# ZHENGXi-git/TC-VIML

Hardware: NVIDIA B200
Metric: linearized_factors_per_s (higher is better)
Workload: dtype f64

## Files before the change

tc-viml_b200/csrc/assemble2.cuh:

```cuda
#pragma once

namespace stream {

constexpr int PMAX = 12;
constexpr int FMAXP = 4096;
constexpr int PT = 64;
constexpr int PT_MAX = 512;
constexpr int TASK_T = 180;
constexpr int TASK_F = 24;
constexpr int LTASK = 32;
constexpr int AW = 4;
constexpr int LACC_W = 14;
constexpr int STAGE_D = 1024;
constexpr int LACC_D = TASK_F * LACC_W;
constexpr int WORK_D = STAGE_D + LACC_D + 192;

struct PlanPtrs {
  int4* hdr;
  int4* tasks;
  uint32_t* slots;
  uint32_t* finfo;
  uint32_t* lslots;
  int* any_irregular;
};

__host__ __device__ inline int task_base(int a0_rel, int w, int F) { return a0_rel / 64 + w * (F / TASK_F + PMAX + 4); }

__device__ __forceinline__ int warp_incl_scan(int v, int lane) {
#pragma unroll
  for (int d = 1; d < 32; d <<= 1) {
    const int t = __shfl_up_sync(0xffffffffu, v, d);
    if (lane >= d) v += t;
  }
  return v;
}

__global__ void __launch_bounds__(PT_MAX) plan_kernel(LinearizeArgs A, PlanPtrs PL) {
  extern __shared__ __align__(16) unsigned char plan_raw[];
  __shared__ int gcount[PMAX + 2], grun[PMAX + 2], lcount[PMAX + 1], lrun[PMAX + 1];
  __shared__ int s_bad, s_big, s_ntasks, s_nlslots;
  const int tid = threadIdx.x, lane = tid & 31, warp = tid >> 5, w = blockIdx.x;
  const int P = A.P, F = A.F, NTH = (int)blockDim.x;
  uint32_t* fmask = reinterpret_cast<uint32_t*>(plan_raw);
  uint32_t* fanchor = fmask + F;
  uint32_t* cexcl = fanchor + F;
  uint16_t* ford = reinterpret_cast<uint16_t*>(cexcl + F + 1);
  uint16_t* fid = ford + ((F + 1) & ~1);
  const int a0 = A.pf_window_offset[w], nf = A.pf_window_offset[w + 1] - a0;
  const int b0 = A.NL > 0 ? A.lf_window_offset[w] : 0, nl = A.NL > 0 ? A.lf_window_offset[w + 1] - b0 : 0;
  const int a0r = a0 - (int)A.pf_begin, b0r = b0 - (int)A.lf_begin;
  for (int f = tid; f < F; f += NTH) fmask[f] = 0u, fanchor[f] = 0xffu;
  for (int e = tid; e < F * P; e += NTH) fid[e] = 0xffff;
  if (tid < PMAX + 2) gcount[tid] = 0;
  if (tid < PMAX + 1) lcount[tid] = 0;
  if (tid == 0) s_bad = s_big = (nf > 65534 || nl > 65534 || nf < 0 || nl < 0) ? 1 : 0, s_ntasks = 0, s_nlslots = 0;
  __syncthreads();
  const int nfs = s_big ? 0 : nf;
  for (int k = tid; k < nfs; k += NTH) {
    const uint32_t ix = A.pf_idx[a0 + k];
    const int i = ix & 0xff, j = (ix >> 8) & 0xff, l = ix >> 16;
    if (i >= P || j >= P || l >= F || i == j) {
      s_bad = 1;
      continue;
    }
    const uint32_t old = atomicOr(&fmask[l], 1u << j);
    const uint32_t an = atomicCAS(&fanchor[l], 0xffu, (uint32_t)i);
    if (((old >> j) & 1u) || (an != 0xffu && an != (uint32_t)i)) s_bad = 1;
    fid[l * P + j] = (uint16_t)k;
  }
  __syncthreads();
  if (s_bad) {
    if (tid == 0) {
      PL.hdr[w] = make_int4(0, 0, 1, 0);
      atomicOr(PL.any_irregular, 1);
    }
    return;
  }
  uint32_t* lsl = PL.lslots + 2 * (size_t)b0r;
  if (warp == 0) {
    for (int f0 = 0; f0 < F; f0 += 32) {
      const int f = f0 + lane;
      const int key = f < F ? (fanchor[f] == 0xffu ? P : (int)fanchor[f]) : 64 + lane;
      const unsigned m = __match_any_sync(0xffffffffu, key);
      if (f < F && (m & ((1u << lane) - 1u)) == 0u) gcount[key] += __popc(m);
      __syncwarp();
    }
    {
      const int c = lane <= P ? gcount[lane] : 0;
      const int inc = warp_incl_scan(c, lane);
      if (lane <= P) grun[lane] = inc - c;
    }
    __syncwarp();
    for (int f0 = 0; f0 < F; f0 += 32) {
      const int f = f0 + lane;
      const int key = f < F ? (fanchor[f] == 0xffu ? P : (int)fanchor[f]) : 64 + lane;
      const unsigned m = __match_any_sync(0xffffffffu, key);
      const int rank = __popc(m & ((1u << lane) - 1u));
      if (f < F) ford[grun[key] + rank] = (uint16_t)f;
      __syncwarp();
      if (f < F && rank == 0) grun[key] += __popc(m);
      __syncwarp();
    }
    int carry = 0;
    for (int p0 = 0; p0 < F; p0 += 32) {
      const int p = p0 + lane;
      const int c = p < F ? __popc(fmask[ford[p]]) : 0;
      const int inc = warp_incl_scan(c, lane);
      if (p < F) cexcl[p] = (uint32_t)(carry + inc - c);
      carry += __shfl_sync(0xffffffffu, inc, 31);
    }
    if (lane == 0) cexcl[F] = (uint32_t)carry;
    __syncwarp();
    const int tb = task_base(a0r, w, F);
    int pos = 0, t = 0;
    bool at_group_start = true;
    while (pos < F) {
      const int p = pos + lane;
      const int c = p < F ? (int)(cexcl[p + 1] - cexcl[p]) : 0x10000;
      const int inc = warp_incl_scan(c, lane);
      const unsigned okm = __ballot_sync(0xffffffffu, inc <= TASK_T && p < F && lane < TASK_F);
      int n = okm == 0xffffffffu ? 32 : __ffs(~okm) - 1;
      n = max(n, 1);
      n = min(n, F - pos);
      const int an = p < F ? (fanchor[ford[p]] == 0xffu ? P : (int)fanchor[ford[p]]) : -1;
      const unsigned same = __ballot_sync(0xffffffffu, an == __shfl_sync(0xffffffffu, an, 0));
      const int na = same == 0xffffffffu ? 33 : __ffs(~same) - 1;
      int excl = 0;
      if (na <= n) {
        n = na;
        excl = at_group_start ? 1 : 0;
        at_group_start = true;
      } else {
        at_group_start = false;
      }
      if (lane == 0) PL.tasks[tb + t] = make_int4(2 * (int)cexcl[pos], 0, pos, n | (excl << 16));
      pos += n, ++t;
    }
    if (lane == 0) s_ntasks = t;
  } else if (warp == 1 && nl > 0) {
    bool bad = false;
    for (int k0 = 0; k0 < nl; k0 += 32) {
      const int k = k0 + lane;
      int key = k < nl ? A.lf_frame[b0 + k] : 64 + lane;
      if (k < nl && (key < 0 || key >= P)) bad = true, key = 96 + lane;
      const unsigned m = __match_any_sync(0xffffffffu, key);
      if (k < nl && key < P && (m & ((1u << lane) - 1u)) == 0u) lcount[key] += __popc(m);
      __syncwarp();
    }
    if (__any_sync(0xffffffffu, bad)) {
      if (lane == 0) s_bad = 1;
    } else {
      const int c = lane < P ? ((lcount[lane] + 1) & ~1) : 0;
      const int inc = warp_incl_scan(c, lane);
      if (lane < P) {
        lrun[lane] = inc - c;
        if (lcount[lane] & 1) lsl[inc - 1] = 0xffffu | ((uint32_t)lane << 16);
      }
      if (lane == 31) s_nlslots = inc;
      __syncwarp();
      for (int k0 = 0; k0 < nl; k0 += 32) {
        const int k = k0 + lane;
        const int key = k < nl ? A.lf_frame[b0 + k] : 64 + lane;
        const unsigned m = __match_any_sync(0xffffffffu, key);
        const int rank = __popc(m & ((1u << lane) - 1u));
        if (k < nl) lsl[lrun[key] + rank] = (uint32_t)k | ((uint32_t)key << 16);
        __syncwarp();
        if (k < nl && rank == 0) lrun[key] += __popc(m);
        __syncwarp();
      }
    }
  }
  __syncthreads();
  if (s_bad) {
    if (tid == 0) {
      PL.hdr[w] = make_int4(0, 0, 1, 0);
      atomicOr(PL.any_irregular, 1);
    }
    return;
  }
  const int tb = task_base(a0r, w, F), nt = s_ntasks;
  uint32_t* sl_w = PL.slots + 2 * (size_t)a0r;
  for (int t = warp; t < nt; t += NTH / 32) {
    int4 tk = PL.tasks[tb + t];
    const int p = tk.z + lane;
    const bool on = lane < (tk.w & 0xffff);
    const int l = on ? ford[p] : 0;
    const uint32_t m = on ? fmask[l] : 0u;
    const int an = (on && m) ? (int)fanchor[l] : 0xff;
    if (on) PL.finfo[(size_t)w * F + p] = (uint32_t)l | (m << 16) | ((uint32_t)(an & 15) << 28);
    uint32_t* sl = sl_w + tk.x;
    int off = 0;
    const unsigned lt = (1u << lane) - 1u;
    unsigned im = __reduce_or_sync(0xffffffffu, an < P ? 1u << an : 0u);
    while (im) {
      const int i = __ffs(im) - 1;
      im &= im - 1;
      unsigned jm = __reduce_or_sync(0xffffffffu, an == i ? m : 0u);
      while (jm) {
        const int j = __ffs(jm) - 1;
        jm &= jm - 1;
        const bool mine = an == i && ((m >> j) & 1u);
        const unsigned b = __ballot_sync(0xffffffffu, mine);
        const int n = __popc(b);
        const uint32_t key = ((uint32_t)i << 21) | ((uint32_t)j << 25);
        if (mine) sl[off + __popc(b & lt)] = (uint32_t)fid[l * P + j] | ((uint32_t)lane << 16) | key;
        if ((n & 1) && lane == 0) sl[off + n] = 0xffffu | key;
        off += (n + 1) & ~1;
      }
    }
    if (lane == 0) PL.tasks[tb + t].y = off;
  }
  if (tid == 0) PL.hdr[w] = make_int4(nt, s_nlslots, 0, 0);
}

enum Kind { K_LL = 0, K_HH, K_LH, K_LE, K_HE, K_EE, K_BL, K_BH, K_BE, K_NKIND };

struct Tables {
  uint32_t seg[128];
  uint32_t lo[64];
  uint32_t ee[32];
  uint32_t line[32];
};

constexpr uint32_t tab_entry(int R, int C, int kind, int off, bool neg) {
  const int tile = (R < 8 && C < 8) ? 0 : (R < 8 ? 1 : 2);
  return 0x80000000u | (uint32_t)(tile * 64 + (R & 7) * 8 + (C & 7)) | ((uint32_t)kind << 8) | ((uint32_t)off << 12) |
         (neg ? (1u << 18) : 0u);
}

constexpr int col_type(int c) { return c < 3 ? 0 : (c < 6 ? 1 : (c < 9 ? 2 : (c < 15 ? 3 : 4))); }
constexpr int col_sub(int c) { return c < 3 ? c : (c < 6 ? c - 3 : (c < 9 ? c - 6 : (c < 15 ? c - 9 : 0))); }

constexpr Tables make_tables() {
  Tables T{};
  int ns = 0, nlo = 0, nli = 0, nee = 0;
  constexpr int kind_order[K_NKIND] = {K_LL, K_LE, K_BL, K_EE, K_BE, K_HH, K_HE, K_BH, K_LH};
  for (int ko = 0; ko < K_NKIND; ++ko)
    for (int off = 0; off < 36; ++off) {
      const int kind = kind_order[ko];
      const bool vec = kind >= K_BL;
      if (vec && off >= 6) continue;
      const int dr = vec ? off : off / 6, dc = vec ? 0 : off % 6;
      for (int R = 0; R < 16; ++R)
        for (int C = R; C < 16; ++C) {
          const int tr = col_type(R), tc = col_type(C), r = col_sub(R), c = col_sub(C);
          bool hit = false, neg = false;
          if (tr == 0 && tc == 0) {
            if (kind == K_LL || kind == K_HH) hit = dr == r && dc == c;
            if (kind == K_LH) hit = dr == r && dc == c, neg = true;
          } else if (tr == 0 && tc == 1) {
            if (kind == K_LL) hit = dr == r && dc == 3 + c;
            if (kind == K_LH) hit = dr == 3 + c && dc == r, neg = true;
          } else if (tr == 0 && tc == 2) {
            if (kind == K_LH) hit = dr == r && dc == 3 + c;
            if (kind == K_HH) hit = dr == r && dc == 3 + c, neg = true;
          } else if (tr == 0 && tc == 3) {
            if (kind == K_LE) hit = dr == r && dc == c;
            if (kind == K_HE) hit = dr == r && dc == c, neg = true;
          } else if (tr == 0 && tc == 4) {
            if (kind == K_BL) hit = dr == r;
            if (kind == K_BH) hit = dr == r, neg = true;
          } else if (tr == 1 && tc == 1) {
            if (kind == K_LL) hit = dr == 3 + r && dc == 3 + c;
          } else if (tr == 1 && tc == 2) {
            if (kind == K_LH) hit = dr == 3 + r && dc == 3 + c;
          } else if (tr == 1 && tc == 3) {
            if (kind == K_LE) hit = dr == 3 + r && dc == c;
          } else if (tr == 1 && tc == 4) {
            if (kind == K_BL) hit = dr == 3 + r;
          } else if (tr == 2 && tc == 2) {
            if (kind == K_HH) hit = dr == 3 + r && dc == 3 + c;
          } else if (tr == 2 && tc == 3) {
            if (kind == K_HE) hit = dr == 3 + r && dc == c;
          } else if (tr == 2 && tc == 4) {
            if (kind == K_BH) hit = dr == 3 + r;
          } else if (tr == 3 && tc == 3) {
            if (kind == K_EE) hit = dr == r && dc == c;
          } else if (tr == 3 && tc == 4) {
            if (kind == K_BE) hit = dr == r;
          }
          if (!hit) continue;
          const bool per_segment = kind == K_HH || kind == K_LH || kind == K_HE || kind == K_BH;
          if (per_segment) {
            T.seg[ns++] = tab_entry(R, C, kind, off, neg);
          } else if (kind == K_EE || kind == K_BE) {
            T.ee[nee++] = tab_entry(R, C, kind, off, neg);
          } else {
            T.lo[nlo++] = tab_entry(R, C, kind, off, neg);
          }
        }
    }
  for (int r = 0; r < 6; ++r)
    for (int c = r; c < 6; ++c) T.line[nli++] = tab_entry(r, c, K_LL, r * 6 + c, false);
  for (int r = 0; r < 6; ++r) T.line[nli++] = tab_entry(r, 6, K_BL, r, false);
  return T;
}
__device__ const Tables g_tables = make_tables();
static_assert(make_tables().seg[95] != 0u && make_tables().seg[96] == 0u, "63 hi-role + 33 (lo, hi) per-segment destinations = three full rounds");
static_assert(make_tables().lo[62] != 0u && make_tables().lo[63] == 0u, "63 per-anchor destinations");
static_assert(make_tables().ee[26] != 0u && make_tables().ee[27] == 0u, "27 extrinsic destinations");
static_assert(make_tables().line[26] != 0u && make_tables().line[27] == 0u, "27 line destinations");


__device__ __forceinline__ void dmma(double& d0, double& d1, double a, double b) {
  asm volatile("mma.sync.aligned.m8n8k4.row.col.f64.f64.f64.f64 {%0,%1}, {%2}, {%3}, {%0,%1};"
               : "+d"(d0), "+d"(d1)
               : "d"(a), "d"(b));
}

__device__ __forceinline__ int blk(int br, int bc, int NB) { return br * NB - (br * (br - 1)) / 2 + (bc - br); }

__device__ __forceinline__ int swz(int f) { return ((f & 1) << 2) ^ ((f >> 1) & 3); }

struct Dest {
  int src;
  int off;
  int kind;
  unsigned sign;
};
__device__ __forceinline__ Dest decode(uint32_t e) {
  Dest d;
  d.src = (e >> 31) ? (int)(e & 0xff) : -1;
  d.off = (e >> 12) & 63;
  d.kind = (e >> 8) & 15;
  d.sign = ((e >> 18) & 1u) << 31;
  return d;
}
template <int ROUNDS>
__device__ __forceinline__ void scatter(const double* __restrict__ patch, const Dest* tab, double* __restrict__ Hc,
                                        int mybase, bool store_lh = false) {
  double v[ROUNDS];
  double* dst[ROUNDS];
#pragma unroll
  for (int r = 0; r < ROUNDS; ++r) {
    const int base = __shfl_sync(0xffffffffu, mybase, tab[r].kind);
    dst[r] = Hc + base + tab[r].off;
    const double x = patch[tab[r].src >= 0 ? tab[r].src : 0];
    v[r] = __hiloint2double(__double2hiint(x) ^ (int)tab[r].sign, __double2loint(x));
  }
#pragma unroll
  for (int r = 0; r < ROUNDS; ++r) {
    if (tab[r].src >= 0) {
      if (store_lh && tab[r].kind == K_LH) *dst[r] = v[r];
      else atomicAdd(dst[r], v[r]);
    }
  }
}

__device__ __forceinline__ int kind_base(int rs, int cs, bool isb, int lo, int hi, int NB, int boff) {
  const int e = NB - 1;
  const int x = rs == 0 ? lo : (rs == 1 ? hi : e), y = cs == 0 ? lo : (cs == 1 ? hi : e);
  return isb ? boff + 6 * x : blk(x, y, NB) * 36;
}

__device__ __forceinline__ void put_patch(double* __restrict__ patch, int lane, const double (&G)[6]) {
  double2* p2 = reinterpret_cast<double2*>(patch);
  const int o = (lane >> 2) * 4 + (lane & 3);
  p2[o] = make_double2(G[0], G[1]);
  p2[32 + o] = make_double2(G[2], G[3]);
  p2[64 + o] = make_double2(G[4], G[5]);
}

template <bool MODE_A>
__global__ void __maxnreg__(168) assemble_kernel(LinearizeArgs A, PlanPtrs PL, int use_tma) {
  extern __shared__ __align__(16) unsigned char asm_raw[];
  __shared__ int s_next;
  constexpr int NT = AW * 32;
  const int tid = threadIdx.x, lane = tid & 31, warp = tid >> 5, w = blockIdx.x;
  const int P = A.P, F = A.F, D = A.D, NB = P + 1;
  const int nblk = NB * (NB + 1) / 2, boff = nblk * 36;
  const int hc_n = (boff + D + 1) & ~1;
  const int cstride = P * kPoseCache + kExCache;
  double* __restrict__ Hc = reinterpret_cast<double*>(asm_raw);
  double* __restrict__ cache = Hc + hc_n;
  double* __restrict__ work0 = cache + cstride;
  double* __restrict__ stage = work0 + warp * WORK_D;
  double* __restrict__ lacc = stage + STAGE_D;
  double* __restrict__ patch = lacc + LACC_D;

  const int4 hdr = PL.hdr[w];
  const int a0 = A.pf_window_offset[w];
  const int b0 = A.NL > 0 ? A.lf_window_offset[w] : 0;
  double* __restrict__ Hpp = A.out.H_pp + (size_t)w * D * D;
  double* __restrict__ Hlp = A.out.H_lp + (size_t)w * F * D;
  double* __restrict__ Hll = A.out.H_ll + (size_t)w * F;
  double* __restrict__ bp = A.out.b_p + (size_t)w * D;
  double* __restrict__ bl = A.out.b_l + (size_t)w * F;
  const double2* __restrict__ gc = reinterpret_cast<const double2*>(A.cache + (size_t)w * cstride);
  double2 cpre[3];
#pragma unroll
  for (int q = 0; q < 3; ++q) cpre[q] = tid + q * NT < cstride / 2 ? gc[tid + q * NT] : make_double2(0.0, 0.0);
  uint32_t traw[7];
#pragma unroll
  for (int r = 0; r < 3; ++r) traw[r] = g_tables.seg[32 * r + lane];
#pragma unroll
  for (int r = 0; r < 2; ++r) traw[3 + r] = g_tables.lo[32 * r + lane];
  traw[5] = g_tables.ee[lane], traw[6] = g_tables.line[lane];
  if (hdr.z) {
    for (int e = tid; e < D * D; e += NT) Hpp[e] = 0.0;
    for (int e = tid; e < F * D; e += NT) Hlp[e] = 0.0;
    for (int e = tid; e < F; e += NT) Hll[e] = 0.0, bl[e] = 0.0;
    for (int e = tid; e < D; e += NT) bp[e] = 0.0;
    return;
  }
  {
    double2* z = reinterpret_cast<double2*>(Hc);
    for (int e = tid; e < hc_n / 2; e += NT) z[e] = make_double2(0.0, 0.0);
    double2* c2 = reinterpret_cast<double2*>(cache);
#pragma unroll
    for (int q = 0; q < 3; ++q)
      if (tid + q * NT < cstride / 2) c2[tid + q * NT] = cpre[q];
    for (int e = tid + 3 * NT; e < cstride / 2; e += NT) c2[e] = gc[e];
  }
  if (tid == 0) s_next = 0;
  Dest tab_seg[3], tab_lo[2], tab_ee[1], tab_line[1];
#pragma unroll
  for (int r = 0; r < 3; ++r) tab_seg[r] = decode(traw[r]);
#pragma unroll
  for (int r = 0; r < 2; ++r) tab_lo[r] = decode(traw[3 + r]);
  tab_ee[0] = decode(traw[5]);
  tab_line[0] = decode(traw[6]);
  const int kb_rs = lane < K_NKIND ? (0x24904 >> (2 * lane)) & 3 : 0, kb_cs = lane < K_NKIND ? (0xA94 >> (2 * lane)) & 3 : 0;
  const bool kb_isb = lane >= K_BL && lane < K_NKIND;
  __syncthreads();

  const int ntask = hdr.x, nlsl = hdr.y, nltask = (nlsl + LTASK - 1) / LTASK;
  const int tb = task_base(a0 - (int)A.pf_begin, w, F);
  const uint32_t* __restrict__ sl_w = PL.slots + 2 * (size_t)(a0 - (int)A.pf_begin);
  const uint32_t* __restrict__ lsl_w = PL.lslots + 2 * (size_t)(b0 - (int)A.lf_begin);
  const int g = lane >> 2, kk = lane & 3;
  const int gx = g ^ ((kk >> 1) << 2);
  const double* __restrict__ frag0 = stage + (kk >> 1) * 32 + (kk & 1);
  const unsigned full = 0xffffffffu;
  const int upr = 3 * NB;
  const int ru1 = 32 + (lane & 7), rb0 = (lane * 11) >> 5, rb1 = (ru1 * 43) >> 7;
  const int rp0 = lane - 3 * rb0, rp1 = ru1 - 3 * rb1;

  double E[2] = {0.0, 0.0};
  for (;;) {
    int t = 0;
    if (lane == 0) t = atomicAdd(&s_next, 1);
    t = __shfl_sync(full, t, 0);
    if (t >= ntask + nltask) break;
    if (t < ntask) {
      const int4 tk = PL.tasks[tb + t];
      const int n_slots = tk.y, n_feats = tk.w & 0xffff;
      const bool excl = (tk.w >> 16) != 0;
      const uint32_t fi = lane < n_feats ? PL.finfo[(size_t)w * F + tk.z + lane] : 0u;
      {
        double2* z = reinterpret_cast<double2*>(lacc);
        for (int q = lane; q < LACC_D / 2; q += 32) z[q] = make_double2(0.0, 0.0);
      }
      __syncwarp();
      const uint32_t* __restrict__ sl = sl_w + tk.x;
      double G[6] = {0, 0, 0, 0, 0, 0}, R[4] = {0, 0, 0, 0};
      uint32_t nsw = lane < n_slots ? sl[lane] : 0xffffu;
      for (int c0 = 0; c0 < n_slots; c0 += 32) {
        const uint32_t sw_ = nsw;
        nsw = c0 + 32 + lane < n_slots ? sl[c0 + 32 + lane] : 0xffffu;
        const bool valid = (sw_ & 0xffffu) != 0xffffu;
        const int lf = (sw_ >> 16) & 31;
        {
          const int i = (sw_ >> 21) & 15, j = (sw_ >> 25) & 15;
          const int l = __shfl_sync(full, fi, lf) & 0xffff;
          PointJac J;
          if (valid) {
            const int64_t k = (int64_t)a0 + (sw_ & 0xffffu);
            const double4 ob = reinterpret_cast<const double4*>(A.pf_obs)[k];
            const double piz = A.pf_pts_i_z ? A.pf_pts_i_z[k] : 1.0;
            const double lam = A.inv_depth[(size_t)w * F + l];
            eval_point(A, cache, i, j, lam, ob.x, ob.y, piz, ob.z, ob.w, J);
            if (MODE_A) {
              if (A.out.pf_residual) reinterpret_cast<double2*>(A.out.pf_residual)[k] = make_double2(J.r[0], J.r[1]);
              if (A.out.pf_jac_pose_i) store_jac7(A.out.pf_jac_pose_i + 14 * k, J.a);
              if (A.out.pf_jac_pose_j) store_jac7(A.out.pf_jac_pose_j + 14 * k, J.b);
              if (A.out.pf_jac_ex) store_jac7(A.out.pf_jac_ex + 14 * k, J.c);
              if (A.out.pf_jac_feat) reinterpret_cast<double2*>(A.out.pf_jac_feat)[k] = make_double2(J.d[0], J.d[1]);
            }
            double2* row = reinterpret_cast<double2*>(Hlp + (size_t)l * D + 6 * j);
            row[0] = make_double2(J.d[0] * J.b[0][0] + J.d[1] * J.b[1][0], J.d[0] * J.b[0][1] + J.d[1] * J.b[1][1]);
            row[1] = make_double2(J.d[0] * J.b[0][2] + J.d[1] * J.b[1][2], J.d[0] * J.b[0][3] + J.d[1] * J.b[1][3]);
            row[2] = make_double2(J.d[0] * J.b[0][4] + J.d[1] * J.b[1][4], J.d[0] * J.b[0][5] + J.d[1] * J.b[1][5]);
          } else {
#pragma unroll
            for (int c = 0; c < 6; ++c) J.a[0][c] = J.a[1][c] = J.b[0][c] = J.b[1][c] = J.c[0][c] = J.c[1][c] = 0.0;
            J.r[0] = J.r[1] = J.d[0] = J.d[1] = 0.0;
          }
          {
            const bool swp = i > j;
            const int sx = swz(lane);
            double2* rec = reinterpret_cast<double2*>(stage) + lane * 16;
#pragma unroll
            for (int c = 0; c < 6; ++c) rec[c ^ sx] = swp ? make_double2(J.b[0][c], J.b[1][c]) : make_double2(J.a[0][c], J.a[1][c]);
#pragma unroll
            for (int c = 0; c < 3; ++c)
              rec[(6 + c) ^ sx] = swp ? make_double2(J.a[0][3 + c], J.a[1][3 + c]) : make_double2(J.b[0][3 + c], J.b[1][3 + c]);
#pragma unroll
            for (int c = 0; c < 6; ++c) rec[(9 + c) ^ sx] = make_double2(J.c[0][c], J.c[1][c]);
            rec[15 ^ sx] = make_double2(J.r[0], J.r[1]);
          }
          {
            const unsigned grp = __match_any_sync(full, valid ? lf : 32 + lane);
            const int rank = __popc(grp & ((1u << lane) - 1u));
            const int rounds = __reduce_max_sync(full, valid ? __popc(grp) : 0);
            double v[LACC_W];
#pragma unroll
            for (int c = 0; c < 6; ++c) {
              v[c] = J.d[0] * J.a[0][c] + J.d[1] * J.a[1][c];
              v[6 + c] = J.d[0] * J.c[0][c] + J.d[1] * J.c[1][c];
            }
            v[12] = J.d[0] * J.d[0] + J.d[1] * J.d[1];
            v[13] = J.d[0] * J.r[0] + J.d[1] * J.r[1];
            double2* __restrict__ la = reinterpret_cast<double2*>(lacc + lf * LACC_W);
            for (int r = 0; r < rounds; ++r) {
              if (valid && rank == r) {
#pragma unroll
                for (int c = 0; c < LACC_W / 2; ++c) {
// ... 4 lines not shown
              }
              __syncwarp();
            }
          }
        }
        __syncwarp();
        const uint32_t key = sw_ >> 21;
        uint32_t nk = __shfl_down_sync(full, key, 1);
        const uint32_t nk31 = __shfl_sync(full, nsw >> 21, 0);
        if (lane == 31) nk = nk31;
        if (c0 + lane + 1 >= n_slots) nk = 0xffffffffu;
        const unsigned bnd = __ballot_sync(full, key != nk);
        const int nks = min(16, (n_slots - c0) >> 1);
        int s = 0;
        while (s < nks) {
          const unsigned rem = bnd >> (2 * s + 1);
          const int q_end = rem ? ((__ffs(rem) - 1) >> 1) : 32;
          const bool ends = s + q_end < nks;
          const int s_end = ends ? s + q_end + 1 : nks;
#pragma unroll 2
          for (; s < s_end; ++s) {
            const double* __restrict__ p = frag0 + s * 64 + 2 * (gx ^ (s & 3));
            const double u0 = p[0], u1 = p[16];
            dmma(G[0], G[1], u0, u0);
            dmma(G[2], G[3], u0, u1);
            dmma(G[4], G[5], u1, u1);
          }
          if (ends) {
            const int la_ = 2 * s - 2;
            const uint32_t kseg = __shfl_sync(full, key, la_), knext = __shfl_sync(full, nk, la_ + 1);
            const int si = kseg & 15, sj = (kseg >> 4) & 15;
            const int lo = min(si, sj), hi = max(si, sj);
            const int mybase = kind_base(kb_rs, kb_cs, kb_isb, lo, hi, NB, boff);
            put_patch(patch, lane, G);
            __syncwarp();
            scatter<3>(patch, tab_seg, Hc, mybase, excl);
#pragma unroll
            for (int q = 0; q < 4; ++q) R[q] += G[q], G[q] = 0.0;
            E[0] += G[4], E[1] += G[5], G[4] = G[5] = 0.0;
            const bool lo_ends = knext == 0xffffffffu || min((int)(knext & 15), (int)((knext >> 4) & 15)) != lo;
            if (lo_ends) {
              __syncwarp();
              {
                const double R6[6] = {R[0], R[1], R[2], R[3], 0.0, 0.0};
                put_patch(patch, lane, R6);
              }
              __syncwarp();
              scatter<2>(patch, tab_lo, Hc, mybase);
#pragma unroll
              for (int q = 0; q < 4; ++q) R[q] = 0.0;
            }
            __syncwarp();
          }
        }
        __syncwarp();
      }
      for (int f = 0; f < n_feats; ++f) {
        const uint32_t info = __shfl_sync(full, fi, f);
        const int l = info & 0xffff;
        const uint32_t m = (info >> 16) & 0xfffu;
        const int an = m ? (int)(info >> 28) : -1;
        double2* __restrict__ dst = reinterpret_cast<double2*>(Hlp + (size_t)l * D);
        const double2* __restrict__ la = reinterpret_cast<const double2*>(lacc + f * LACC_W);
        const bool ia = rb0 == an, ie = rb0 == P;
        double2 v = la[ia ? rp0 : 3 + rp0];
        if (!(ia || ie)) v = make_double2(0.0, 0.0);
        if ((ia || ie || !((m >> rb0) & 1u)) && lane < upr) dst[lane] = v;
      }
      if (upr > 32) {
        const int fs = lane >> 3;
        for (int f0 = 0; f0 < n_feats; f0 += 4) {
          const int f = f0 + fs;
          const uint32_t info = __shfl_sync(full, fi, f & 31);
          const int l = info & 0xffff;
          const uint32_t m = (info >> 16) & 0xfffu;
          const int an = m ? (int)(info >> 28) : -1;
          const bool ia = rb1 == an, ie = rb1 == P;
          if (f < n_feats && ru1 < upr) {
            double2 v = reinterpret_cast<const double2*>(lacc + f * LACC_W)[ia ? rp1 : 3 + rp1];
            if (!(ia || ie)) v = make_double2(0.0, 0.0);
            if (ia || ie || !((m >> rb1) & 1u)) reinterpret_cast<double2*>(Hlp + (size_t)l * D)[ru1] = v;
          }
        }
      }
      if (lane < n_feats) {
        const int l = fi & 0xffff;
        Hll[l] = lacc[lane * LACC_W + 12];
        bl[l] = lacc[lane * LACC_W + 13];
      }
      __syncwarp();
    } else {
      const int t0 = (t - ntask) * LTASK, n_slots = min(LTASK, nlsl - t0);
      const uint32_t sw_ = lane < n_slots ? lsl_w[t0 + lane] : 0xffffu;
      const bool valid = (sw_ & 0xffffu) != 0xffffu;
      const int frame = (sw_ >> 16) & 0xff;
      {
        LineJac J;
        if (valid) {
          const int64_t k = (int64_t)b0 + (sw_ & 0xffffu);
          double g9[9];
#pragma unroll
          for (int c = 0; c < 9; ++c) g9[c] = A.lf_geom[(size_t)c * A.NL_stride + k];
          eval_line(A, cache, frame, g9, J);
          if (MODE_A) {
            if (A.out.lf_residual) reinterpret_cast<double2*>(A.out.lf_residual)[k] = make_double2(J.r[0], J.r[1]);
            if (A.out.lf_jac_pose) store_jac7(A.out.lf_jac_pose + 14 * k, J.a);
          }
        } else {
#pragma unroll
          for (int c = 0; c < 6; ++c) J.a[0][c] = J.a[1][c] = 0.0;
          J.r[0] = J.r[1] = 0.0;
        }
        const int sx = swz(lane);
        double2* rec = reinterpret_cast<double2*>(stage) + lane * 16;
#pragma unroll
        for (int c = 0; c < 6; ++c) rec[c ^ sx] = make_double2(J.a[0][c], J.a[1][c]);
        rec[6 ^ sx] = make_double2(J.r[0], J.r[1]);
        rec[7 ^ sx] = make_double2(0.0, 0.0);
      }
      __syncwarp();
      const uint32_t key = sw_ >> 16;
      uint32_t nk = __shfl_down_sync(full, key, 1);
      if (lane + 1 >= n_slots) nk = 0xffffffffu;
      const unsigned bnd = __ballot_sync(full, key != nk);
      const int nks = n_slots >> 1;
      double G[6] = {0, 0, 0, 0, 0, 0};
      int s = 0;
      while (s < nks) {
        const unsigned rem = bnd >> (2 * s + 1);
        const int s_end = min(nks, s + ((__ffs(rem) - 1) >> 1) + 1);
        for (; s < s_end; ++s) {
          const double u0 = frag0[s * 64 + 2 * (gx ^ (s & 3))];
          dmma(G[0], G[1], u0, u0);
        }
        const int fr = __shfl_sync(full, key, 2 * s - 2) & 0xff;
        const int mybase = kind_base(kb_rs, kb_cs, kb_isb, fr, fr, NB, boff);
        put_patch(patch, lane, G);
        __syncwarp();
        scatter<1>(patch, tab_line, Hc, mybase);
        G[0] = G[1] = 0.0;
        __syncwarp();
      }
    }
  }
  {
    const int mybase = kind_base(kb_rs, kb_cs, kb_isb, 0, 0, NB, boff);
    const double E6[6] = {0.0, 0.0, 0.0, 0.0, E[0], E[1]};
    __syncwarp();
    put_patch(patch, lane, E6);
    __syncwarp();
    scatter<1>(patch, tab_ee, Hc, mybase);
  }
  __syncthreads();
  double* __restrict__ Hf = work0;
  const bool staged = D * D + D <= AW * WORK_D;
  const bool aligned16 = use_tma != 0;
  if (!staged) {
    Hf = Hpp;
    use_tma = 0;
  }
  if (!staged && !aligned16) {
    for (int e = tid; e < D * D; e += NT) {
      const int r = e / D, c = e - r * D;
      const int br = r / 6, bc = c / 6, rr = r - 6 * br, cc = c - 6 * bc;
      const int lo = min(br, bc), hi = max(br, bc);
      const bool tr = br > bc || (br == bc && rr > cc);
      int a = tr ? cc : rr, b = tr ? rr : cc;
      if (lo != hi && hi < NB - 1 && a < 3 && b < a) { const int t = a; a = b, b = t; }
      Hpp[e] = Hc[blk(lo, hi, NB) * 36 + a * 6 + b];
    }
  } else {
    double2* __restrict__ Hf2 = reinterpret_cast<double2*>(Hf);
    const int Dh = D / 2;
    int br = 0, row0 = 0, rown = NB;
    for (int e = tid; e < nblk * 18; e += NT) {
      const int q = (e * 3641) >> 16, k = e - 18 * q;
      const int rr = (k * 11) >> 5, cp = k - 3 * rr, cc = 2 * cp;
      while (q >= row0 + rown) row0 += rown, --rown, ++br;
      const int bc = br + (q - row0);
      const double* __restrict__ sb = Hc + q * 36;
      if (br != bc) {
        const bool pp = bc < NB - 1;
        auto at = [&](int a, int b) { return sb[(pp && a < 3 && b < a) ? b * 6 + a : a * 6 + b]; };
        Hf2[(6 * br + rr) * Dh + 3 * bc + cp] = make_double2(at(rr, cc), at(rr, cc + 1));
        Hf2[(6 * bc + rr) * Dh + 3 * br + cp] = make_double2(at(cc, rr), at(cc + 1, rr));
      } else {
        Hf2[(6 * br + rr) * Dh + 3 * bc + cp] =
            make_double2(rr <= cc ? sb[rr * 6 + cc] : sb[cc * 6 + rr], rr <= cc + 1 ? sb[rr * 6 + cc + 1] : sb[(cc + 1) * 6 + rr]);
      }
    }
  }
  if (staged) {
    for (int e = tid; e < D; e += NT) Hf[D * D + e] = Hc[boff + e];
  } else {
    for (int e = tid; e < D; e += NT) bp[e] = Hc[boff + e];
  }
  if (use_tma) {
    asm volatile("fence.proxy.async.shared::cta;" ::: "memory");
    __syncthreads();
    if (tid == 0) {
      const uint32_t s0 = (uint32_t)__cvta_generic_to_shared(Hf);
      asm volatile("cp.async.bulk.global.shared::cta.bulk_group [%0], [%1], %2;" ::"l"(Hpp), "r"(s0), "r"((uint32_t)(D * D * 8))
                   : "memory");
      asm volatile("cp.async.bulk.global.shared::cta.bulk_group [%0], [%1], %2;" ::"l"(bp), "r"(s0 + (uint32_t)(D * D * 8)),
                   "r"((uint32_t)(D * 8))
                   : "memory");
      asm volatile("cp.async.bulk.commit_group;" ::: "memory");
      asm volatile("cp.async.bulk.wait_group.read 0;" ::: "memory");
    }
  } else if (staged) {
    __syncthreads();
    for (int e = tid; e < D * D; e += NT) Hpp[e] = Hf[e];
    for (int e = tid; e < D; e += NT) bp[e] = Hf[D * D + e];
  }
}

template <bool MODE_A>
__global__ void __launch_bounds__(128) irregular_kernel(LinearizeArgs A, PlanPtrs PL) {
  if (!*PL.any_irregular) return;
  const int cstride = A.P * kPoseCache + kExCache;
  for (int w = blockIdx.x; w < A.W; w += gridDim.x) {
    if (!PL.hdr[w].z) continue;
    const double* cw = A.cache + (size_t)w * cstride;
    const int a0 = A.pf_window_offset[w], a1 = A.pf_window_offset[w + 1];
    for (int64_t k = a0 + threadIdx.x; k < a1; k += blockDim.x) {
      const uint32_t pk = A.pf_idx[k];
      const int i = pk & 0xff, j = (pk >> 8) & 0xff, f = pk >> 16;
      if (i >= A.P || j >= A.P || f >= A.F) continue;
      const double4 ob = reinterpret_cast<const double4*>(A.pf_obs)[k];
      const double piz = A.pf_pts_i_z ? A.pf_pts_i_z[k] : 1.0;
      PointJac J;
      eval_point(A, cw, i, j, A.inv_depth[(size_t)w * A.F + f], ob.x, ob.y, piz, ob.z, ob.w, J);
      if (MODE_A) {
        if (A.out.pf_residual) reinterpret_cast<double2*>(A.out.pf_residual)[k] = make_double2(J.r[0], J.r[1]);
        if (A.out.pf_jac_pose_i) store_jac7(A.out.pf_jac_pose_i + 14 * k, J.a);
        if (A.out.pf_jac_pose_j) store_jac7(A.out.pf_jac_pose_j + 14 * k, J.b);
        if (A.out.pf_jac_ex) store_jac7(A.out.pf_jac_ex + 14 * k, J.c);
        if (A.out.pf_jac_feat) reinterpret_cast<double2*>(A.out.pf_jac_feat)[k] = make_double2(J.d[0], J.d[1]);
      }
      point_atomics(A, w, i, j, f, J, true, false);
    }
    if (A.NL > 0) {
      const int b0 = A.lf_window_offset[w], b1 = A.lf_window_offset[w + 1];
      for (int64_t k = b0 + threadIdx.x; k < b1; k += blockDim.x) {
        const int frame = A.lf_frame[k];
        if (frame < 0 || frame >= A.P) continue;
        double g9[9];
#pragma unroll
        for (int c = 0; c < 9; ++c) g9[c] = A.lf_geom[(size_t)c * A.NL_stride + k];
        LineJac J;
        eval_line(A, cw, frame, g9, J);
        if (MODE_A) {
          if (A.out.lf_residual) reinterpret_cast<double2*>(A.out.lf_residual)[k] = make_double2(J.r[0], J.r[1]);
          if (A.out.lf_jac_pose) store_jac7(A.out.lf_jac_pose + 14 * k, J.a);
        }
        line_atomics(A, w, frame, J);
      }
    }
  }
}

}
```

tc-viml_b200/csrc/linearize_kernels.cu:

```cuda
#include <cstdlib>
#include <vector>

#include "common.cuh"

namespace {

__device__ __forceinline__ void quat_to_rot(double w, double x, double y, double z, double* R) {
  const double tx = 2.0 * x, ty = 2.0 * y, tz = 2.0 * z;
  const double twx = tx * w, twy = ty * w, twz = tz * w;
  const double txx = tx * x, txy = ty * x, txz = tz * x;
  const double tyy = ty * y, tyz = tz * y, tzz = tz * z;
  R[0] = 1.0 - (tyy + tzz);
  R[1] = txy - twz;
  R[2] = txz + twy;
  R[3] = txy + twz;
  R[4] = 1.0 - (txx + tzz);
  R[5] = tyz - twx;
  R[6] = txz - twy;
  R[7] = tyz + twx;
  R[8] = 1.0 - (txx + tyy);
}

__device__ __forceinline__ void mul_AtBt(const double* A, const double* B, double* C) {
#pragma unroll
// ... 336 lines not shown
          if (c != r) atomicAdd(H + (size_t)(oe + c) * D + oe + r, v[n]);
          ++n;
        }
#pragma unroll
      for (int r = 0; r < 6; ++r) atomicAdd(bp + oe + r, v[21 + r]);
    }
  }
  if (!live) return;
  double* Hl = A.out.H_lp + ((size_t)w * A.F + f) * D;
  atomic_block(H, D, oi, oi, J.a, J.a, true);
  atomic_block(H, D, oi, oj, J.a, J.b, false);
  atomic_block(H, D, oi, oe, J.a, J.c, false);
  atomic_block(H, D, oj, oj, J.b, J.b, true);
  atomic_block(H, D, oj, oe, J.b, J.c, false);
  if (!warp_window) atomic_block(H, D, oe, oe, J.c, J.c, true);
#pragma unroll
  for (int r = 0; r < 6; ++r) {
    atomicAdd(bp + oi + r, J.a[0][r] * J.r[0] + J.a[1][r] * J.r[1]);
    atomicAdd(bp + oj + r, J.b[0][r] * J.r[0] + J.b[1][r] * J.r[1]);
    if (!warp_window) atomicAdd(bp + oe + r, J.c[0][r] * J.r[0] + J.c[1][r] * J.r[1]);
    atomicAdd(Hl + oi + r, J.a[0][r] * J.d[0] + J.a[1][r] * J.d[1]);
    atomicAdd(Hl + oj + r, J.b[0][r] * J.d[0] + J.b[1][r] * J.d[1]);
    atomicAdd(Hl + oe + r, J.c[0][r] * J.d[0] + J.c[1][r] * J.d[1]);
  }
  atomicAdd(A.out.H_ll + (size_t)w * A.F + f, J.d[0] * J.d[0] + J.d[1] * J.d[1]);
  atomicAdd(A.out.b_l + (size_t)w * A.F + f, J.d[0] * J.r[0] + J.d[1] * J.r[1]);
}

__device__ __forceinline__ void line_atomics(const LinearizeArgs& A, int w, int frame, const LineJac& J) {
  const int D = A.D;
  double* H = A.out.H_pp + (size_t)w * D * D;
  double* bp = A.out.b_p + (size_t)w * D;
  const int of = 6 * frame;
  atomic_block(H, D, of, of, J.a, J.a, true);
#pragma unroll
  for (int r = 0; r < 6; ++r) atomicAdd(bp + of + r, J.a[0][r] * J.r[0] + J.a[1][r] * J.r[1]);
}

template <bool MODE_A, bool MODE_B>
#ifndef VIML_POINTS_MINB
#define VIML_POINTS_MINB 4
#endif
__global__ void __launch_bounds__(128, MODE_B ? 2 : VIML_POINTS_MINB) points_kernel(LinearizeArgs A) {
  __shared__ double2 stage[MODE_A ? 4 * 7 * 32 : 1];
  const int64_t k_raw = A.pf_begin + blockIdx.x * (int64_t)blockDim.x + threadIdx.x;
  const int64_t k_end = A.pf_begin + A.NP;
  const int lane = threadIdx.x & 31;
  const int64_t k_warp = k_raw - lane;
  if (k_warp >= k_end) return;
  const int nvalid = (int)min((int64_t)32, k_end - k_warp);
  const int64_t k = min(k_raw, k_end - 1);
  const bool live = k_raw < k_end;
  const int w = find_window_warp(A.pf_window_offset, A.W, k, k_warp);
  const uint32_t pk = A.pf_idx[k];
  const int i = pk & 0xff, j = (pk >> 8) & 0xff, f = pk >> 16;
  const double4 ob = reinterpret_cast<const double4*>(A.pf_obs)[k];
  const double piz = A.pf_pts_i_z ? A.pf_pts_i_z[k] : 1.0;
  const double lam = A.inv_depth[(size_t)w * A.F + f];
  const double* cw = A.cache + (size_t)w * (A.P * kPoseCache + kExCache);
  PointJac J;
  eval_point(A, cw, i, j, lam, ob.x, ob.y, piz, ob.z, ob.w, J);
  if (MODE_A) {
    double2* st = stage + (threadIdx.x >> 5) * 7 * 32;
    if (live && A.out.pf_residual) reinterpret_cast<double2*>(A.out.pf_residual)[k] = make_double2(J.r[0], J.r[1]);
    if (A.out.pf_jac_pose_i) store_jac7_coalesced(st, A.out.pf_jac_pose_i + 14 * k_warp, J.a, lane, nvalid);
    if (A.out.pf_jac_pose_j) store_jac7_coalesced(st, A.out.pf_jac_pose_j + 14 * k_warp, J.b, lane, nvalid);
    if (A.out.pf_jac_ex) store_jac7_coalesced(st, A.out.pf_jac_ex + 14 * k_warp, J.c, lane, nvalid);
    if (live && A.out.pf_jac_feat) reinterpret_cast<double2*>(A.out.pf_jac_feat)[k] = make_double2(J.d[0], J.d[1]);
  }
  if (MODE_B) {
    const bool warp_window = __all_sync(0xffffffffu, w == __shfl_sync(0xffffffffu, w, 0));
    point_atomics(A, w, i, j, f, J, live, warp_window);
  }
}

template <bool MODE_A, bool MODE_B>
__global__ void __launch_bounds__(128) lines_kernel(LinearizeArgs A) {
  __shared__ double2 stage[MODE_A ? 4 * 7 * 32 : 1];
  const int64_t k_raw = A.lf_begin + blockIdx.x * (int64_t)blockDim.x + threadIdx.x;
  const int64_t k_end = A.lf_begin + A.NL;
  const int lane = threadIdx.x & 31;
  const int64_t k_warp = k_raw - lane;
  if (k_warp >= k_end) return;
  const int nvalid = (int)min((int64_t)32, k_end - k_warp);
  const int64_t k = min(k_raw, k_end - 1);
  const bool live = k_raw < k_end;
  const int w = find_window_warp(A.lf_window_offset, A.W, k, k_warp);
  const int frame = A.lf_frame[k];
  double g9[9];
#pragma unroll
  for (int c = 0; c < 9; ++c) g9[c] = A.lf_geom[(size_t)c * A.NL_stride + k];
  const double* cw = A.cache + (size_t)w * (A.P * kPoseCache + kExCache);
  LineJac J;
  eval_line(A, cw, frame, g9, J);
  if (MODE_A) {
    if (live && A.out.lf_residual) reinterpret_cast<double2*>(A.out.lf_residual)[k] = make_double2(J.r[0], J.r[1]);
    if (A.out.lf_jac_pose)
      store_jac7_coalesced(stage + (threadIdx.x >> 5) * 7 * 32, A.out.lf_jac_pose + 14 * k_warp, J.a, lane, nvalid);
  }
  if (MODE_B && live) line_atomics(A, w, frame, J);
}

__global__ void __launch_bounds__(256) pack_upper_kernel(int D, const double* __restrict__ S, double* __restrict__ Sp) {
  const double* __restrict__ s = S + (size_t)blockIdx.x * D * D;
  double* __restrict__ o = Sp + (size_t)blockIdx.x * ((size_t)D * (D + 1) / 2);
  for (int e = blockIdx.y * blockDim.x + threadIdx.x; e < D * D; e += gridDim.y * blockDim.x) {
    const int r = e / D, c = e - r * D;
    if (c >= r) o[(size_t)r * D - ((size_t)r * (r - 1)) / 2 + c - r] = s[e];
  }
}

#include "assemble2.cuh"
#include "gn_kernels.cuh"

}

int viml_launch_linearize(viml_ctx* ctx, const LinearizeArgs& a) {
  cudaStream_t st = ctx->stream;
  const bool modeA = (a.flags & VIML_OUT_RESIDUAL_JACOBIAN) != 0;
  const bool modeB = (a.flags & (VIML_OUT_HB | VIML_OUT_SCHUR)) != 0;
  const size_t plan_smem = (size_t)a.F * 8 + ((size_t)a.F + 1) * 4 + (((size_t)a.F + 1) & ~(size_t)1) * 2 + (size_t)a.F * a.P * 2 + 16;
  const bool fast = modeB && a.P <= stream::PMAX && a.F <= stream::FMAXP && plan_smem <= 200 * 1024 && !ctx->force_generic;
  stream::PlanPtrs PL{};
  if (fast) {
    const size_t n_tasks = (size_t)a.NP / 64 + (size_t)a.W * (a.F / stream::TASK_F + stream::PMAX + 4) + 2;
    auto pad = [](size_t b) { return DeviceArena::padded(b); };
    VIML_TRY_CUDA(ctx, ctx->scratch3.reserve(pad((size_t)a.W * 16) + pad(n_tasks * 16) + pad((size_t)a.NP * 8 + 8) +
                                             pad((size_t)a.W * a.F * 4 + 4) + pad((size_t)a.NL * 8 + 8) + pad(4)));
    PL.hdr = ctx->scratch3.take<int4>((size_t)a.W);
    PL.tasks = ctx->scratch3.take<int4>(n_tasks);
    PL.slots = ctx->scratch3.take<uint32_t>((size_t)a.NP * 2 + 2);
    PL.finfo = ctx->scratch3.take<uint32_t>((size_t)a.W * a.F + 1);
    PL.lslots = ctx->scratch3.take<uint32_t>((size_t)a.NL * 2 + 2);
    PL.any_irregular = ctx->scratch3.take<int>(1);
    VIML_TRY_CUDA(ctx, cudaEventRecord(ctx->ev_fork, st));
    VIML_TRY_CUDA(ctx, cudaStreamWaitEvent(ctx->aux_stream, ctx->ev_fork, 0));
    VIML_TRY_CUDA(ctx, cudaMemsetAsync(PL.any_irregular, 0, 4, ctx->aux_stream));
    VIML_TRY_CUDA(ctx, cudaFuncSetAttribute(stream::plan_kernel, cudaFuncAttributeMaxDynamicSharedMemorySize, (int)plan_smem));
    {
      LaunchScope ls(ctx, K_PLAN, ctx->aux_stream);
      stream::plan_kernel<<<a.W, a.F > 512 ? stream::PT_MAX : stream::PT, plan_smem, ctx->aux_stream>>>(a, PL);
    }
    VIML_TRY_CUDA(ctx, cudaEventRecord(ctx->ev_join, ctx->aux_stream));
  }
  {
    const int64_t total = (int64_t)a.W * (a.P + 1);
    LaunchScope ls(ctx, K_PREP);
    prep_windows_kernel<<<(unsigned)((total + 127) / 128), 128, 0, st>>>(a);
  }
  if (fast) {
    VIML_TRY_CUDA(ctx, cudaStreamWaitEvent(st, ctx->ev_join, 0));
    const int NB = a.P + 1, nblk = NB * (NB + 1) / 2;
    const size_t smem = ((size_t)((nblk * 36 + a.D + 1) & ~1) + (size_t)a.P * kPoseCache + kExCache + (size_t)stream::AW * stream::WORK_D) * 8;
    const int use_tma = ((((uintptr_t)a.out.H_pp) | ((uintptr_t)a.out.b_p)) & 15) == 0 ? 1 : 0;
    VIML_TRY_CUDA(ctx, cudaFuncSetAttribute(stream::assemble_kernel<true>, cudaFuncAttributeMaxDynamicSharedMemorySize, (int)smem));
    VIML_TRY_CUDA(ctx, cudaFuncSetAttribute(stream::assemble_kernel<false>, cudaFuncAttributeMaxDynamicSharedMemorySize, (int)smem));
    {
      LaunchScope ls(ctx, K_ASSEMBLE);
      if (modeA) stream::assemble_kernel<true><<<a.W, stream::AW * 32, smem, st>>>(a, PL, use_tma);
      else stream::assemble_kernel<false><<<a.W, stream::AW * 32, smem, st>>>(a, PL, use_tma);
    }
    {
      const int grid = a.W < 4 * ctx->sm_count ? a.W : 4 * ctx->sm_count;
      LaunchScope ls(ctx, K_IRREGULAR);
      if (modeA) stream::irregular_kernel<true><<<grid, 128, 0, st>>>(a, PL);
      else stream::irregular_kernel<false><<<grid, 128, 0, st>>>(a, PL);
    }
  } else {
    if (modeB) {
      const size_t W = a.W, D = a.D, F = a.F;
      VIML_TRY_CUDA(ctx, cudaMemsetAsync(a.out.H_pp, 0, W * D * D * sizeof(double), st));
      VIML_TRY_CUDA(ctx, cudaMemsetAsync(a.out.H_lp, 0, W * F * D * sizeof(double), st));
      VIML_TRY_CUDA(ctx, cudaMemsetAsync(a.out.H_ll, 0, W * F * sizeof(double), st));
      VIML_TRY_CUDA(ctx, cudaMemsetAsync(a.out.b_p, 0, W * D * sizeof(double), st));
      VIML_TRY_CUDA(ctx, cudaMemsetAsync(a.out.b_l, 0, W * F * sizeof(double), st));
    }
    if (a.NP > 0) {
      const unsigned grid = (unsigned)((a.NP + 127) / 128);
      LaunchScope ls(ctx, K_POINTS);
      if (modeA && modeB) points_kernel<true, true><<<grid, 128, 0, st>>>(a);
      else if (modeA) points_kernel<true, false><<<grid, 128, 0, st>>>(a);
      else if (modeB) points_kernel<false, true><<<grid, 128, 0, st>>>(a);
    }
    if (a.NL > 0) {
      const unsigned grid = (unsigned)((a.NL + 127) / 128);
      LaunchScope ls(ctx, K_LINES);
      if (modeA && modeB) lines_kernel<true, true><<<grid, 128, 0, st>>>(a);
      else if (modeA) lines_kernel<true, false><<<grid, 128, 0, st>>>(a);
      else if (modeB) lines_kernel<false, true><<<grid, 128, 0, st>>>(a);
    }
  }
  if (a.flags & VIML_OUT_SCHUR) {
    const double eps = 1e-8;
    double* S = a.out.S;
    if (a.flags & VIML_S_PACKED) {
      VIML_TRY_CUDA(ctx, ctx->s_full.reserve(DeviceArena::padded((size_t)a.W * a.D * a.D * 8)));
      S = ctx->s_full.take<double>((size_t)a.W * a.D * a.D);
    }
    viml_launch_schur(ctx, a.W, a.F, a.D, a.out.H_pp, a.out.H_lp, a.out.H_ll, a.out.b_p, a.out.b_l, S, a.out.g, eps);
    if (a.flags & VIML_S_PACKED) {
      LaunchScope ls(ctx, K_SCHUR);
      const unsigned slices = (unsigned)std::min<int64_t>(((int64_t)a.D * a.D + 256 * 32 - 1) / (256 * 32), 1024);
      pack_upper_kernel<<<dim3((unsigned)a.W, slices), 256, 0, st>>>(a.D, S, a.out.S);
    }
  }
  VIML_TRY_CUDA(ctx, cudaGetLastError());
  return VIML_OK;
}

int viml_launch_expand_obs(viml_ctx* ctx, const LinearizeArgs& a, const void* feat_obs, const void* pf_obs_j, bool f32) {
  if (a.NP == 0) return VIML_OK;
  LaunchScope ls(ctx, K_PREP);
  if (f32) expand_obs_kernel<float2><<<a.W, 128, 0, ctx->stream>>>(a, (const float2*)feat_obs, (const float2*)pf_obs_j);
  else expand_obs_kernel<double2><<<a.W, 128, 0, ctx->stream>>>(a, (const double2*)feat_obs, (const double2*)pf_obs_j);
  VIML_TRY_CUDA(ctx, cudaGetLastError());
  return VIML_OK;
}

int viml_launch_expand_lines(viml_ctx* ctx, const LinearizeArgs& a, const int32_t* lf_map_index, const float* lf_seg2d) {
  if (a.NL == 0) return VIML_OK;
  if (!ctx->map_set || ctx->n_map <= 0) {
    ctx->err = "line factors given by map index need a map (viml_set_map)";
    return VIML_ERR_NOMAP;
  }
  MapFrame mf;
  for (int k = 0; k < 9; ++k) mf.R[k] = ctx->cfg.Rbw[k];
  for (int k = 0; k < 3; ++k) mf.T[k] = ctx->cfg.Tbw[k];
  LaunchScope ls(ctx, K_PREP);
  expand_lines_kernel<<<(unsigned)((a.NL + 127) / 128), 128, 0, ctx->stream>>>(a, ctx->d_map, ctx->n_map, mf, lf_map_index,
                                                                             reinterpret_cast<const float4*>(lf_seg2d));
  VIML_TRY_CUDA(ctx, cudaGetLastError());
  return VIML_OK;
}

int viml_launch_prep(viml_ctx* ctx, const LinearizeArgs& a) {
  const int64_t total = (int64_t)a.W * (a.P + 1);
  LaunchScope ls(ctx, K_PREP);
  prep_windows_kernel<<<(unsigned)((total + 127) / 128), 128, 0, ctx->stream>>>(a);
  VIML_TRY_CUDA(ctx, cudaGetLastError());
  return VIML_OK;
}

int viml_launch_reduced(viml_ctx* ctx, int W, int D, const DenseArgs& dn, const double* S, const double* g, double* Sx, double* gx) {
  LaunchScope ls(ctx, K_GN);
  const int smem = gn::kReducedStage * (int)sizeof(double);
  VIML_TRY_CUDA(ctx, cudaFuncSetAttribute(gn::reduced_kernel, cudaFuncAttributeMaxDynamicSharedMemorySize, smem));
  gn::reduced_kernel<<<W, 256, smem, ctx->stream>>>(D, dn, S, g, Sx, gx);
  VIML_TRY_CUDA(ctx, cudaGetLastError());
  return VIML_OK;
}

constexpr size_t gn_solve_smem(int Dx) {
  const size_t NB = (Dx + 7) / 8;
  return (NB * (NB + 1) / 2 * 64 + NB * 8) * sizeof(double);
}
static_assert(gn_solve_smem(kMaxDx) <= 220 * 1024, "the tiled Cholesky of the largest reduced system must fit in shared memory");

int viml_launch_gn_solve(viml_ctx* ctx, int W, int Dx, double lambda, const double* Sx, const double* gx, double* dx, int32_t* solved,
                         double* cost, const double* lambda_w, const int32_t* running) {
  const size_t smem = gn_solve_smem(Dx);
  LaunchScope ls(ctx, K_GN);
  VIML_TRY_CUDA(ctx, cudaFuncSetAttribute(gn::solve_tiled_kernel<false>, cudaFuncAttributeMaxDynamicSharedMemorySize, (int)smem));
  gn::solve_tiled_kernel<false><<<W, 256, smem, ctx->stream>>>(Dx, lambda, Sx, gx, dx, solved, cost, 0, DenseArgs{}, nullptr, nullptr,
                                                                lambda_w, running);
  VIML_TRY_CUDA(ctx, cudaGetLastError());
  return VIML_OK;
}

int viml_launch_gn_reduced_solve(viml_ctx* ctx, int W, int D, const DenseArgs& dn, const double* S, const double* g, double lambda,
                                 double* dx, int32_t* solved, double* cost, const double* lambda_w, const int32_t* running) {
  const int Dx = D + dn.X, NB = (Dx + 7) / 8;
  const size_t smem = ((size_t)NB * (NB + 1) / 2 * 64 + 3 * (size_t)NB * 8 + gn::kFusedStage) * sizeof(double);
  if (smem > 224 * 1024) return VIML_ERR_UNSUPPORTED;
  LaunchScope ls(ctx, K_GN);
  VIML_TRY_CUDA(ctx, cudaFuncSetAttribute(gn::solve_tiled_kernel<true>, cudaFuncAttributeMaxDynamicSharedMemorySize, (int)smem));
  gn::solve_tiled_kernel<true><<<W, 256, smem, ctx->stream>>>(Dx, lambda, nullptr, nullptr, dx, solved, cost, D, dn, S, g, lambda_w,
                                                               running);
  VIML_TRY_CUDA(ctx, cudaGetLastError());
  return VIML_OK;
}

int viml_launch_gn_update(viml_ctx* ctx, const LinearizeArgs& a, int X, const double* extra_in, const double* dx, const int32_t* solved,
                          double* o_poses, double* o_ex, double* o_dep, double* o_extra, const int32_t* running) {
  LaunchScope ls(ctx, K_GN);
  gn::update_kernel<<<a.W, 128, 0, ctx->stream>>>(a, X, extra_in, dx, solved, o_poses, o_ex, o_dep, o_extra, running);
  VIML_TRY_CUDA(ctx, cudaGetLastError());
  return VIML_OK;
}

int viml_launch_cost(viml_ctx* ctx, const LinearizeArgs& a, const DenseArgs& dn, const double* dx, const int32_t* solved, int slot,
                     double* cost, const int32_t* running) {
  LaunchScope ls(ctx, K_GN);
  gn::cost_kernel<<<a.W, 128, 0, ctx->stream>>>(a, dn, dx, solved, slot, cost, running);
  VIML_TRY_CUDA(ctx, cudaGetLastError());
  return VIML_OK;
}

int viml_launch_solve_policy(viml_ctx* ctx, int W, const SolveArgs& s, int round) {
  LaunchScope ls(ctx, K_GN);
  gn::policy_kernel<<<W, 128, 0, ctx->stream>>>(s, round);
  VIML_TRY_CUDA(ctx, cudaGetLastError());
  return VIML_OK;
}
```

Measured before the change: 5.511 billion.

## Write Hessian directly to global, batch plan index loads, shrink irregular grid

The plan kernel no longer pre-fills the fid table and now batches four pf_idx loads per thread before the atomic updates, which exposes more memory-level parallelism. The assemble kernel drops the shared-memory staging plus TMA bulk-copy path when outputs are 16-byte aligned, and instead writes the expanded dense Hessian straight to global memory with double2 stores. The irregular kernel grid is reduced from four to one block per SM. Removing the fid initialisation relies on every read entry having been written; removing staging trades a bulk async copy for direct, possibly less coalesced, global writes.

```diff
diff --git a/tc-viml_b200/csrc/assemble2.cuh b/tc-viml_b200/csrc/assemble2.cuh
--- a/tc-viml_b200/csrc/assemble2.cuh
+++ b/tc-viml_b200/csrc/assemble2.cuh
@@ -50,23 +50,30 @@
   const int b0 = A.NL > 0 ? A.lf_window_offset[w] : 0, nl = A.NL > 0 ? A.lf_window_offset[w + 1] - b0 : 0;
   const int a0r = a0 - (int)A.pf_begin, b0r = b0 - (int)A.lf_begin;
   for (int f = tid; f < F; f += NTH) fmask[f] = 0u, fanchor[f] = 0xffu;
-  for (int e = tid; e < F * P; e += NTH) fid[e] = 0xffff;
   if (tid < PMAX + 2) gcount[tid] = 0;
   if (tid < PMAX + 1) lcount[tid] = 0;
   if (tid == 0) s_bad = s_big = (nf > 65534 || nl > 65534 || nf < 0 || nl < 0) ? 1 : 0, s_ntasks = 0, s_nlslots = 0;
   __syncthreads();
   const int nfs = s_big ? 0 : nf;
-  for (int k = tid; k < nfs; k += NTH) {
-    const uint32_t ix = A.pf_idx[a0 + k];
-    const int i = ix & 0xff, j = (ix >> 8) & 0xff, l = ix >> 16;
-    if (i >= P || j >= P || l >= F || i == j) {
-      s_bad = 1;
-      continue;
-    }
-    const uint32_t old = atomicOr(&fmask[l], 1u << j);
-    const uint32_t an = atomicCAS(&fanchor[l], 0xffu, (uint32_t)i);
-    if (((old >> j) & 1u) || (an != 0xffu && an != (uint32_t)i)) s_bad = 1;
-    fid[l * P + j] = (uint16_t)k;
+  for (int k0 = tid; k0 < nfs; k0 += 4 * NTH) {
+    uint32_t ixs[4];
+#pragma unroll
+    for (int u = 0; u < 4; ++u) ixs[u] = k0 + u * NTH < nfs ? A.pf_idx[a0 + k0 + u * NTH] : 0u;
+#pragma unroll
+    for (int u = 0; u < 4; ++u) {
+      const int k = k0 + u * NTH;
+      if (k >= nfs) break;
+      const uint32_t ix = ixs[u];
+      const int i = ix & 0xff, j = (ix >> 8) & 0xff, l = ix >> 16;
+      if (i >= P || j >= P || l >= F || i == j) {
+        s_bad = 1;
+        continue;
+      }
+      const uint32_t old = atomicOr(&fmask[l], 1u << j);
+      const uint32_t an = atomicCAS(&fanchor[l], 0xffu, (uint32_t)i);
+      if (((old >> j) & 1u) || (an != 0xffu && an != (uint32_t)i)) s_bad = 1;
+      fid[l * P + j] = (uint16_t)k;
+    }
   }
   __syncthreads();
   if (s_bad) {
@@ -362,7 +369,7 @@
 }
 
 template <bool MODE_A>
-__global__ void __maxnreg__(168) assemble_kernel(LinearizeArgs A, PlanPtrs PL, int use_tma) {
+__global__ void __maxnreg__(168) assemble_kernel(LinearizeArgs A, PlanPtrs PL, int out_aligned16) {
   extern __shared__ __align__(16) unsigned char asm_raw[];
   __shared__ int s_next;
   constexpr int NT = AW * 32;
@@ -673,13 +680,9 @@
     scatter<1>(patch, tab_ee, Hc, mybase);
   }
   __syncthreads();
-  double* __restrict__ Hf = work0;
-  const bool staged = D * D + D <= AW * WORK_D;
-  const bool aligned16 = use_tma != 0;
-  if (!staged) {
-    Hf = Hpp;
-    use_tma = 0;
-  }
+  const bool aligned16 = out_aligned16 != 0;
+  const bool staged = !aligned16 && D * D + D <= AW * WORK_D;
+  double* __restrict__ Hf = staged ? work0 : Hpp;
   if (!staged && !aligned16) {
     for (int e = tid; e < D * D; e += NT) {
       const int r = e / D, c = e - r * D;
@@ -713,26 +716,11 @@
   }
   if (staged) {
     for (int e = tid; e < D; e += NT) Hf[D * D + e] = Hc[boff + e];
-  } else {
-    for (int e = tid; e < D; e += NT) bp[e] = Hc[boff + e];
-  }
-  if (use_tma) {
-    asm volatile("fence.proxy.async.shared::cta;" ::: "memory");
-    __syncthreads();
-    if (tid == 0) {
-      const uint32_t s0 = (uint32_t)__cvta_generic_to_shared(Hf);
-      asm volatile("cp.async.bulk.global.shared::cta.bulk_group [%0], [%1], %2;" ::"l"(Hpp), "r"(s0), "r"((uint32_t)(D * D * 8))
-                   : "memory");
-      asm volatile("cp.async.bulk.global.shared::cta.bulk_group [%0], [%1], %2;" ::"l"(bp), "r"(s0 + (uint32_t)(D * D * 8)),
-                   "r"((uint32_t)(D * 8))
-                   : "memory");
-      asm volatile("cp.async.bulk.commit_group;" ::: "memory");
-      asm volatile("cp.async.bulk.wait_group.read 0;" ::: "memory");
-    }
-  } else if (staged) {
     __syncthreads();
     for (int e = tid; e < D * D; e += NT) Hpp[e] = Hf[e];
     for (int e = tid; e < D; e += NT) bp[e] = Hf[D * D + e];
+  } else {
+    for (int e = tid; e < D; e += NT) bp[e] = Hc[boff + e];
   }
 }
 
diff --git a/tc-viml_b200/csrc/linearize_kernels.cu b/tc-viml_b200/csrc/linearize_kernels.cu
--- a/tc-viml_b200/csrc/linearize_kernels.cu
+++ b/tc-viml_b200/csrc/linearize_kernels.cu
@@ -512,16 +512,16 @@
     VIML_TRY_CUDA(ctx, cudaStreamWaitEvent(st, ctx->ev_join, 0));
     const int NB = a.P + 1, nblk = NB * (NB + 1) / 2;
     const size_t smem = ((size_t)((nblk * 36 + a.D + 1) & ~1) + (size_t)a.P * kPoseCache + kExCache + (size_t)stream::AW * stream::WORK_D) * 8;
-    const int use_tma = ((((uintptr_t)a.out.H_pp) | ((uintptr_t)a.out.b_p)) & 15) == 0 ? 1 : 0;
+    const int aligned16 = ((((uintptr_t)a.out.H_pp) | ((uintptr_t)a.out.b_p)) & 15) == 0 ? 1 : 0;
     VIML_TRY_CUDA(ctx, cudaFuncSetAttribute(stream::assemble_kernel<true>, cudaFuncAttributeMaxDynamicSharedMemorySize, (int)smem));
     VIML_TRY_CUDA(ctx, cudaFuncSetAttribute(stream::assemble_kernel<false>, cudaFuncAttributeMaxDynamicSharedMemorySize, (int)smem));
     {
       LaunchScope ls(ctx, K_ASSEMBLE);
-      if (modeA) stream::assemble_kernel<true><<<a.W, stream::AW * 32, smem, st>>>(a, PL, use_tma);
-      else stream::assemble_kernel<false><<<a.W, stream::AW * 32, smem, st>>>(a, PL, use_tma);
+      if (modeA) stream::assemble_kernel<true><<<a.W, stream::AW * 32, smem, st>>>(a, PL, aligned16);
+      else stream::assemble_kernel<false><<<a.W, stream::AW * 32, smem, st>>>(a, PL, aligned16);
     }
     {
-      const int grid = a.W < 4 * ctx->sm_count ? a.W : 4 * ctx->sm_count;
+      const int grid = a.W < ctx->sm_count ? a.W : ctx->sm_count;
       LaunchScope ls(ctx, K_IRREGULAR);
       if (modeA) stream::irregular_kernel<true><<<grid, 128, 0, st>>>(a, PL);
       else stream::irregular_kernel<false><<<grid, 128, 0, st>>>(a, PL);
```

New measurement: 5.639 billion (median of 6 runs). 2.3% higher.
